# octavian-ganea/equidock_public

Measured on NVIDIA H100. Metric: protein_pairs_per_sec_iegmn_fwd_kabsch, higher is better.
Workload: dtype f32

## Files before the change

equidock_public_b200/csrc/attn_tc.cu:

```cuda
#include "tc_common.cuh"

namespace eqd {

#ifdef ATTN_PROF
__device__ long long g_attn_prof[16];
#define PROF_MARK(k) do { if (tid == 0 && blockIdx.x == 0) { const long long t_ = clock64(); prof_acc[k] += t_ - prof_t; prof_t = t_; } } while (0)
#else
#define PROF_MARK(k) do { } while (0)
#endif

#define AT_THREADS 256
#define AT_KEYS 64
#define AT_CHUNK_BYTES 8192
#define AT_A_SPLIT 16384
#define AT_LD 68

template <bool X5>
struct AtGroupSmem {
  unsigned char k[2][3][AT_CHUNK_BYTES];
  unsigned char v[2][3][AT_CHUNK_BYTES];
  float red[EQD_TM * 2];
  float x5c[X5 ? 2 : 1][X5 ? AT_KEYS * 16 : 4];
  float red5[X5 ? EQD_TM * 2 * 5 : 4];
};
template <bool X5>
struct AtSmem {
  unsigned char qa[3 * AT_A_SPLIT];
  unsigned char pa[3 * AT_A_SPLIT];
  AtGroupSmem<X5> grp;
  unsigned long long k_bar[2], v_bar[2];
};

template <bool X5>
__global__ void __launch_bounds__(AT_THREADS, 1)
attention_tc_kernel(eqd_graph g, const float* __restrict__ proj, int pw, const unsigned char* __restrict__ kv,
                    long kv_split_stride, const float* __restrict__ x5, float* __restrict__ mu, int ldmu) {
  extern __shared__ __align__(128) unsigned char smem_raw[];
  AtSmem<X5>& S = *reinterpret_cast<AtSmem<X5>*>(smem_raw);
  const int tid = threadIdx.x, q = tid, half = q >> 7, r = q & 127, wgi = tid >> 7;
  AtGroupSmem<X5>& G = S.grp;
  TRACE_START(1);
  if (tid == 0) {
    for (int b = 0; b < 2; ++b) {
      mbar_init(&S.k_bar[b], 1);
      mbar_init(&S.v_bar[b], 1);
    }
    asm volatile("fence.mbarrier_init.release.cluster;" ::: "memory");
  }
  if (q == 0) TRACE_PHASE(1, blockIdx.x, 0, 14);
  __syncthreads();
  if (q == 0) TRACE_PHASE(1, blockIdx.x, 0, 13);
  const unsigned k_saddr = smem_u32(G.k), v_saddr = smem_u32(G.v);
  const unsigned qa_saddr = smem_u32(S.qa), pa_saddr = smem_u32(S.pa);
  float* const dtile = reinterpret_cast<float*>(S.pa);
  unsigned kph[2] = {0, 0}, vph[2] = {0, 0};
  const int B = g.n_pairs;
  const unsigned char* k_g = kv;
  const unsigned char* v_g = kv + 3 * kv_split_stride;

  auto load_chunk = [&](const unsigned char* src, unsigned char (*dst)[AT_CHUNK_BYTES], unsigned long long* bar, int blk0,
                        int x5buf) {
    if (q == 0) {
      const bool with5 = X5 && x5buf >= 0;
      mbar_expect_tx(bar, 3 * AT_CHUNK_BYTES + (with5 ? AT_KEYS * 64 : 0));
#pragma unroll
      for (int s = 0; s < 3; ++s) bulk_g2s(dst[s], src + s * kv_split_stride + (long)blk0 * 1024, AT_CHUNK_BYTES, bar);
      if (with5) bulk_g2s(G.x5c[x5buf], x5 + (long)blk0 * 8 * 16, AT_KEYS * 64, bar);
    }
  };
  auto add_s5 = [&](float (&s)[32], const float* xc, const float (&q5)[5]) {
#pragma unroll
    for (int i = 0; i < 32; ++i) {
      const float* row = xc + (half * 32 + i) * 16;
      const float4 k4 = *reinterpret_cast<const float4*>(row);
      const float k8 = row[8];
      s[i] += q5[0] * k4.x + q5[1] * k4.y + q5[2] * k4.z + q5[3] * k4.w + q5[4] * k8;
    }
  };
  auto gemm_s = [&](int kb_, bool hi_only) {
    float d[32];
    wg_gemm6<64>(d, [&](int sp, int kb) { return a_desc_at<EQD_TM>(qa_saddr, AT_A_SPLIT, wgi, sp, kb); },
                 [&](int sp, int kk) { return b_desc_ex(k_saddr + (kb_ * 3 + sp) * AT_CHUNK_BYTES + kk * 256, 128, 1024); },
                 4, false, hi_only);
    wg_store_d<64>(dtile + wgi * 64 * AT_LD, AT_LD, d, tid & 127);
  };
  auto gemm_pv = [&](int vb_) {
    float d[32];
    wg_gemm6<64, 1>(d, [&](int sp, int kb) { return a_desc_at<EQD_TM>(pa_saddr, AT_A_SPLIT, wgi, sp, kb); },
                    [&](int sp, int kk) { return b_desc_ex(v_saddr + (vb_ * 3 + sp) * AT_CHUNK_BYTES + kk * 2048, 1024, 128); },
                    4, false);
    __syncthreads();
    wg_store_d<64>(dtile + wgi * 64 * AT_LD, AT_LD, d, tid & 127);
  };

#ifdef ATTN_PROF
  __shared__ long long prof_acc[16];
  long long prof_t = clock64();
  if (tid == 0)
    for (int k = 0; k < 16; ++k) prof_acc[k] = 0;
#endif
  for (int tile = blockIdx.x; tile < g.n_node_tiles; tile += gridDim.x) {
    PROF_MARK(15);
    if (q == 0) TRACE_PHASE(1, blockIdx.x, tile, 1);
    const int seg = g.node_tiles[2 * tile], node0 = g.node_tiles[2 * tile + 1];
    const int nvalid = min(EQD_TM, g.seg_ptr[seg + 1] - node0);
    const int pseg = seg < B ? seg + B : seg - B;
    const int j0 = g.seg_ptr[pseg], j1 = g.seg_ptr[pseg + 1];
    const int blk_lo = j0 >> 3, blk_hi = (j1 + 7) >> 3;
    const int nchunks = (blk_hi - blk_lo + 7) >> 3;
    const int node = node0 + r;
    const bool valid = r < nvalid;
    PROF_MARK(0);
    if (nchunks > 0) load_chunk(k_g, G.k[0], &S.k_bar[0], blk_lo, 0);
    float q5[5] = {0.f, 0.f, 0.f, 0.f, 0.f};
    if (X5 && valid) {
#pragma unroll
      for (int e = 0; e < 5; ++e) q5[e] = x5[(long)node * 16 + 10 + e];
    }
    {
      float v[32];
      const float4* sp = reinterpret_cast<const float4*>(proj + (long)node * pw + 128 + half * 32);
#pragma unroll
      for (int c4 = 0; c4 < 8; ++c4) {
        float4 t = valid ? sp[c4] : make_float4(0.f, 0.f, 0.f, 0.f);
        v[c4 * 4] = t.x; v[c4 * 4 + 1] = t.y; v[c4 * 4 + 2] = t.z; v[c4 * 4 + 3] = t.w;
      }
      store_half_split3<EQD_TM>(S.qa, AT_A_SPLIT, r, half * 32, v);
    }
    tc_fence_before();
    __syncthreads();
    PROF_MARK(1);
    float mx = -INFINITY;
    for (int c = 0; c < nchunks; ++c) {
      const int kb_ = c & 1;
      if (q == 0) TRACE_PHASE(1, blockIdx.x, tile, (c << 4) | 2);
      mbar_wait(&S.k_bar[kb_], kph[kb_]);
      kph[kb_] ^= 1;
      PROF_MARK(2);
      if (c + 1 < nchunks) load_chunk(k_g, G.k[kb_ ^ 1], &S.k_bar[kb_ ^ 1], blk_lo + 8 * (c + 1), kb_ ^ 1);
      else load_chunk(k_g, G.k[kb_ ^ 1], &S.k_bar[kb_ ^ 1], blk_lo, kb_ ^ 1);
      if (q == 0) TRACE_PHASE(1, blockIdx.x, tile, (c << 4) | 3);
      gemm_s(kb_, true);
      __syncthreads();
      PROF_MARK(3);
      float s[32];
      tile_ld32f(dtile, AT_LD, r, half * 32, s);
      if (X5) add_s5(s, G.x5c[kb_], q5);
      const int key0 = (blk_lo + 8 * c) * 8 + half * 32;
#pragma unroll
      for (int i = 0; i < 32; ++i) {
        int kn = key0 + i;
        mx = fmaxf(mx, (kn >= j0 && kn < j1) ? s[i] : -INFINITY);
      }
      __syncthreads();
      PROF_MARK(4);
    }
    G.red[r * 2 + half] = mx;
    __syncthreads();
    mx = fmaxf(G.red[r * 2], G.red[r * 2 + 1]);
    float l = 0.f;
    float o_acc[32];
#pragma unroll
    for (int i = 0; i < 32; ++i) o_acc[i] = 0.f;
    if (nchunks > 0) load_chunk(v_g, G.v[0], &S.v_bar[0], blk_lo, -1);
    float o5[5] = {0.f, 0.f, 0.f, 0.f, 0.f};
    for (int c = 0; c < nchunks; ++c) {
      const int kb_ = (nchunks + c) & 1, vb_ = c & 1;
      if (q == 0) TRACE_PHASE(1, blockIdx.x, tile, (c << 4) | 4);
      mbar_wait(&S.k_bar[kb_], kph[kb_]);
      kph[kb_] ^= 1;
      PROF_MARK(5);
      if (c + 1 < nchunks) {
        load_chunk(k_g, G.k[kb_ ^ 1], &S.k_bar[kb_ ^ 1], blk_lo + 8 * (c + 1), kb_ ^ 1);
        load_chunk(v_g, G.v[vb_ ^ 1], &S.v_bar[vb_ ^ 1], blk_lo + 8 * (c + 1), -1);
      }
      if (q == 0) TRACE_PHASE(1, blockIdx.x, tile, (c << 4) | 5);
      gemm_s(kb_, false);
      __syncthreads();
      PROF_MARK(6);
      float s[32];
      tile_ld32f(dtile, AT_LD, r, half * 32, s);
      if (X5) add_s5(s, G.x5c[kb_], q5);
      const int key0 = (blk_lo + 8 * c) * 8 + half * 32;
      float l4[4] = {0.f, 0.f, 0.f, 0.f};
#pragma unroll
      for (int i = 0; i < 32; ++i) {
        int kn = key0 + i;
        float pj = (kn >= j0 && kn < j1) ? expf(s[i] - mx) : 0.f;
        s[i] = pj;
        l4[i & 3] += pj;
        if (X5) {
          const float* row = G.x5c[kb_] + (half * 32 + i) * 16;
          const float4 v4 = *reinterpret_cast<const float4*>(row + 4);
          o5[0] = fmaf(pj, v4.x, o5[0]);
          o5[1] = fmaf(pj, v4.y, o5[1]);
          o5[2] = fmaf(pj, v4.z, o5[2]);
          o5[3] = fmaf(pj, v4.w, o5[3]);
          o5[4] = fmaf(pj, row[9], o5[4]);
        }
      }
      l += (l4[0] + l4[1]) + (l4[2] + l4[3]);
      PROF_MARK(7);
      __syncthreads();
      PROF_MARK(8);
      store_half_split3<EQD_TM>(S.pa, AT_A_SPLIT, r, half * 32, s);
      tc_fence_before();
      __syncthreads();
      PROF_MARK(9);
      if (q == 0) TRACE_PHASE(1, blockIdx.x, tile, (c << 4) | 6);
      mbar_wait(&S.v_bar[vb_], vph[vb_]);
      vph[vb_] ^= 1;
      gemm_pv(vb_);
      __syncthreads();
      if (q == 0) TRACE_PHASE(1, blockIdx.x, tile, (c << 4) | 7);
      PROF_MARK(10);
      {
        float oc[32];
        tile_ld32f(dtile, AT_LD, r, half * 32, oc);
#pragma unroll
        for (int i = 0; i < 32; ++i) o_acc[i] += oc[i];
      }
      __syncthreads();
      PROF_MARK(11);
    }
    G.red[r * 2 + half] = l;
    if (X5) {
#pragma unroll
      for (int e = 0; e < 5; ++e) G.red5[(r * 2 + half) * 5 + e] = o5[e];
    }
    __syncthreads();
    l = G.red[r * 2] + G.red[r * 2 + 1];
    {
      const float inv = l > 0.f ? 1.f / l : 0.f;
      if (X5 && valid && half == 0) {
        float e8[8];
#pragma unroll
        for (int e = 0; e < 5; ++e) e8[e] = (G.red5[r * 10 + e] + G.red5[r * 10 + 5 + e]) * inv;
        e8[5] = e8[6] = e8[7] = 0.f;
        float4* de = reinterpret_cast<float4*>(mu + (long)node * ldmu + 64);
        de[0] = make_float4(e8[0], e8[1], e8[2], e8[3]);
        de[1] = make_float4(e8[4], e8[5], e8[6], e8[7]);
      }
      if (valid) {
        float4* dst = reinterpret_cast<float4*>(mu + (long)node * ldmu + half * 32);
#pragma unroll
        for (int c4 = 0; c4 < 8; ++c4)
          dst[c4] = make_float4(o_acc[c4 * 4] * inv, o_acc[c4 * 4 + 1] * inv, o_acc[c4 * 4 + 2] * inv, o_acc[c4 * 4 + 3] * inv);
      }
    }
    __syncthreads();
    PROF_MARK(12);
  }
#ifdef ATTN_PROF
  if (tid == 0 && blockIdx.x == 0)
    for (int k = 0; k < 16; ++k) g_attn_prof[k] = prof_acc[k];
#endif
  if (q == 0) TRACE_PHASE(1, blockIdx.x, 0xffff, 15);
  TRACE_END(1);
}

}

EQD_TRACE_SETTER(eqd_trace_set_attn)

#ifdef ATTN_PROF
extern "C" int eqd_attn_prof_read(long long* out16) {
  return (int)cudaMemcpyFromSymbol(out16, eqd::g_attn_prof, sizeof(long long) * 16);
}
#endif

template <bool X5>
static int launch_attention_tc(const eqd_graph* g, const float* proj, int pw, const void* kv, const float* x5, float* mu,
                               int ldmu, void* stream) {
  if (reinterpret_cast<uintptr_t>(kv) & 15) return EQD_ERR_BAD_ARG;
  if (g->n_node_tiles <= 0) return EQD_OK;
  size_t smem = sizeof(eqd::AtSmem<X5>) + 128;
  EQD_SET_SMEM((eqd::attention_tc_kernel<X5>), smem);
  int grid = g->n_node_tiles < EQD_SMS ? g->n_node_tiles : EQD_SMS;
  long split_stride = (long)((g->n_nodes + 7) / 8 + 8) * 1024;
  eqd::attention_tc_kernel<X5><<<grid, AT_THREADS, smem, (cudaStream_t)stream>>>(
      *g, proj, pw, reinterpret_cast<const unsigned char*>(kv), split_stride, x5, mu, ldmu);
  EQD_CUDA_LAUNCH_CHECK();
  return EQD_OK;
}

extern "C" int eqd_attention_tc(const eqd_graph* g, const float* proj, const void* kv, float* mu, void* stream) {
  if (!g || !proj || !kv || !mu) return EQD_ERR_BAD_ARG;
  return launch_attention_tc<false>(g, proj, 320, kv, nullptr, mu, EQD_HID, stream);
}

extern "C" int eqd_attention_tc0(const eqd_graph* g, const float* proj, const void* kv, const float* x5, float* mu,
                                 void* stream) {
  if (!g || !proj || !kv || !x5 || !mu) return EQD_ERR_BAD_ARG;
  if (reinterpret_cast<uintptr_t>(x5) & 15) return EQD_ERR_BAD_ARG;
  return launch_attention_tc<true>(g, proj, 128 + 3 * 72, kv, x5, mu, EQD_H0_PAD, stream);
}
```

equidock_public_b200/csrc/edge_stage_tc.cu:

```cuda
#include "tc_common.cuh"

namespace eqd {
#define TC_WGS 3
#define TC_THREADS (128 * TC_WGS)
#define TC_ROWS 64
#define TC_MAX_TN 32
#define TC_LD 72
#define TC_W_BYTES 67584
#define TC_W1_SPLIT 6144
#define TC_W23_BASE 18432
#define TC_W23_SPLIT 16384
#define TC_HE_FLOATS (TC_ROWS * EQD_EDGE_FEATS + 16)
#define TC_A_SPLIT 6144

struct __align__(128) TcWgSmem {
  unsigned char a[3 * TC_A_SPLIT];
  float msg[TC_ROWS * TC_LD];
  float he[TC_HE_FLOATS];
  double xs[2][TC_ROWS * 6];
  double xm[TC_ROWS * 3];
  double phi[TC_ROWS];
  int src[2][TC_ROWS];
  int dst[2][TC_ROWS];
  int rp[2][TC_MAX_TN + 4];
  unsigned long long he_bar;
};

struct EdgeConsts {
  float ln_g[64], ln_b[64], b2[64], b3[64], w4[64];
};

struct TcSmem {
  unsigned char w[TC_W_BYTES];
  TcWgSmem wg[TC_WGS];
  EdgeConsts cst;
  unsigned long long w_bar;
};

__device__ __forceinline__ float chain_val(const float (&v)[32], const float (&pv)[32], int h, int ch, int c4, int e) {
  const int i = 4 * (4 * ch + (c4 >> 1)) + 2 * h + e;
  const bool own = ((c4 & 1) == 0) == ((threadIdx.x & 2) == 0);
  return own ? v[i] : pv[i];
}

__global__ void __launch_bounds__(TC_THREADS, 1)
edge_stage_tc_kernel(eqd_graph g, eqd_layer_params p, const __grid_constant__ EdgeConsts cst_p,
                     const float* __restrict__ proj, const double* __restrict__ x_in, const double* __restrict__ x_orig,
                     float* __restrict__ aggr, double* __restrict__ x_out, int* __restrict__ status, int tn) {
  extern __shared__ __align__(128) unsigned char smem_raw[];
  TcSmem& S = *reinterpret_cast<TcSmem*>(smem_raw);
  const int tid = threadIdx.x, wgi = tid >> 7, t = tid & 127, r = t & 63, half = t >> 6;
  const int warp = t >> 5, lane = t & 31;
  TcWgSmem& W = S.wg[wgi];
  const EdgeConsts& cst = S.cst;
  const int bar = 1 + wgi;
  const int pw = 128 + 3 * p.dhp;
  const int ntiles = (g.n_nodes + tn - 1) / tn;
  const float slope = p.leaky_slope;

  TRACE_START(0);
  if (tid == 0) {
    mbar_init(&S.w_bar, 1);
    for (int w = 0; w < TC_WGS; ++w) mbar_init(&S.wg[w].he_bar, 1);
    asm volatile("fence.mbarrier_init.release.cluster;" ::: "memory");
    mbar_expect_tx(&S.w_bar, TC_W_BYTES);
    bulk_g2s(S.w, p.w_edge_tc, TC_W_BYTES, &S.w_bar);
  }
  for (int i = tid; i < 5 * 64; i += TC_THREADS) (&S.cst.ln_g[0])[i] = (&cst_p.ln_g[0])[i];
  __syncthreads();
  mbar_wait(&S.w_bar, 0);
  unsigned he_phase = 0;
  const unsigned w_saddr = smem_u32(S.w), a_saddr = smem_u32(W.a);
  auto a_desc = [&](int sp, int kb) { return a_desc_at<TC_ROWS>(a_saddr, TC_A_SPLIT, 0, sp, kb); };

  auto prefetch = [&](int tile, int buf, int e0, int e1, int& off_l, int& n_l, int& off_r) {
    const int n0 = tile * tn, nn = min(tn, g.n_nodes - n0);
// ... 351 lines not shown
```

equidock_public_b200/csrc/proj_tc.cu:

```cuda
#include "tc_common.cuh"

namespace eqd {

#define PJ_LD 68

template <bool L0>
struct PjCfg {
  static constexpr int R = L0 ? 64 : 128;
  static constexpr int THREADS = 2 * R;
  static constexpr int KB = L0 ? 5 : 4;
  static constexpr int GROUP_BYTES = 64 * KB * 16 * 2 * 3;
  static constexpr int SPLIT_BYTES = 64 * KB * 16 * 2;
  static constexpr int X_SPLIT_BYTES = 16 * KB * 16 * 2;
  static constexpr int W_BYTES = 5 * GROUP_BYTES + (L0 ? 3 * X_SPLIT_BYTES : 0);
  static constexpr int A_SPLIT_BYTES = R * KB * 32;
  static constexpr int NGROUPS = L0 ? 6 : 5;
};

struct PjConsts { float b[336]; };

template <bool L0>
struct PjSmem {
  unsigned char w[PjCfg<L0>::W_BYTES];
  unsigned char a[3 * PjCfg<L0>::A_SPLIT_BYTES];
// ... 98 lines not shown
#pragma unroll
      for (int c = 0; c < 32; ++c) {
        float t = v[c] + cst.b[grp * 64 + half * 32 + c];
        v[c] = act ? lrelu(t, slope) : t;
      }
      if (grp < 3 || kv == nullptr) {
        if (L0) {
          if (valid) {
            float4* o = reinterpret_cast<float4*>(proj + (long)node * pw + grp * 64 + half * 32);
#pragma unroll
            for (int c4 = 0; c4 < 8; ++c4) o[c4] = make_float4(v[c4 * 4], v[c4 * 4 + 1], v[c4 * 4 + 2], v[c4 * 4 + 3]);
          }
        } else {
          float* sc = S.d + r * PJ_LD + half * 32;
#pragma unroll
          for (int c4 = 0; c4 < 8; ++c4)
            *reinterpret_cast<float4*>(sc + c4 * 4) = make_float4(v[c4 * 4], v[c4 * 4 + 1], v[c4 * 4 + 2], v[c4 * 4 + 3]);
          __syncwarp();
          float* o = proj + (long)(node0 + wrow0) * pw + grp * 64 + half * 32 + (lane & 7) * 4;
#pragma unroll
          for (int i = 0; i < 8; ++i) {
            const int row = i * 4 + (lane >> 3);
            float4 t = *reinterpret_cast<const float4*>(S.d + (wrow0 + row) * PJ_LD + half * 32 + (lane & 7) * 4);
            if (node0 + wrow0 + row < n_nodes) *reinterpret_cast<float4*>(o + (long)row * pw) = t;
          }
        }
      }
      if (valid && grp >= 3 && kv != nullptr)
        store_kv_blocks(kv + (long)(grp - 3) * 3 * kv_split_stride, kv_split_stride, node, half, v);
      __syncthreads();
    }
    __syncthreads();
  }
  TRACE_END(2);
}

__global__ void kv_blocks_kernel(int n_nodes, const float* __restrict__ proj, int pw, int koff, int voff,
                                 unsigned char* __restrict__ kv, long kv_split_stride) {
  int idx = blockIdx.x * blockDim.x + threadIdx.x;
  int node = idx >> 2, which = (idx >> 1) & 1, half = idx & 1;
  if (node >= n_nodes) return;
  const float4* src = reinterpret_cast<const float4*>(proj + (long)node * pw + (which ? voff : koff) + half * 32);
  float v[32];
#pragma unroll
  for (int c4 = 0; c4 < 8; ++c4) {
    float4 t = src[c4];
    v[c4 * 4] = t.x; v[c4 * 4 + 1] = t.y; v[c4 * 4 + 2] = t.z; v[c4 * 4 + 3] = t.w;
  }
  store_kv_blocks(kv + (long)which * 3 * kv_split_stride, kv_split_stride, node, half, v);
}

}

EQD_TRACE_SETTER(eqd_trace_set_proj)

extern "C" size_t eqd_kv_blocks_bytes(int32_t n_nodes) {
  return (size_t)6 * ((size_t)(n_nodes + 7) / 8 + 8) * 1024;
}

template <bool L0>
static int launch_project_tc(const eqd_graph* g, const eqd_layer* p_l, const float* h, int ldh, float* proj, int pw,
                             void* kv, float* x5, void* stream) {
  const eqd_layer_params* p = &p_l->dev;
  if (!(p->leaky_slope >= 0.f && p->leaky_slope <= 1.f)) return EQD_ERR_UNSUPPORTED;
  if (!p->w_proj_tc || (reinterpret_cast<uintptr_t>(p->w_proj_tc) & 15)) return EQD_ERR_BAD_ARG;
  if (g->n_nodes <= 0) return EQD_OK;
  eqd::PjConsts cst;
  memset(&cst, 0, sizeof(cst));
  memcpy(&cst, p_l->consts.proj_bias, 320 * sizeof(float));
  int ntiles = (g->n_nodes + eqd::PjCfg<L0>::R - 1) / eqd::PjCfg<L0>::R;
  size_t smem = sizeof(eqd::PjSmem<L0>) + 128;
  EQD_SET_SMEM((eqd::project_tc_kernel<L0>), smem);
  int grid = ntiles < EQD_SMS ? ntiles : EQD_SMS;
  long split_stride = (long)((g->n_nodes + 7) / 8 + 8) * 1024;
  eqd::project_tc_kernel<L0><<<grid, eqd::PjCfg<L0>::THREADS, smem, (cudaStream_t)stream>>>(
      g->n_nodes, *p, cst, h, ldh, proj, pw, reinterpret_cast<unsigned char*>(kv), split_stride, x5);
  EQD_CUDA_LAUNCH_CHECK();
  return EQD_OK;
}

extern "C" int eqd_project_tc(const eqd_graph* g, const eqd_layer* p_l, const float* h, float* proj, void* kv,
                              void* stream) {
  const eqd_layer_params* p = p_l ? &p_l->dev : nullptr;
  if (!g || !p || !h || !proj) return EQD_ERR_BAD_ARG;
  if (p->dh != 64 || p->dhp != 64) return EQD_ERR_UNSUPPORTED;
  return launch_project_tc<false>(g, p_l, h, EQD_HID, proj, 320, kv, nullptr, stream);
}

extern "C" int eqd_project_tc0(const eqd_graph* g, const eqd_layer* p_l, const float* h0, float* proj, void* kv,
                               float* x5, void* stream) {
  const eqd_layer_params* p = p_l ? &p_l->dev : nullptr;
  if (!g || !p || !h0 || !proj || !kv || !x5) return EQD_ERR_BAD_ARG;
  if (p->dh != 69 || p->dhp != 72) return EQD_ERR_UNSUPPORTED;
  return launch_project_tc<true>(g, p_l, h0, EQD_H0_PAD, proj, 128 + 3 * 72, kv, x5, stream);
}

extern "C" int eqd_kv_blocks(const eqd_graph* g, const float* proj, int32_t pw, int32_t koff, int32_t voff, void* kv,
                             void* stream) {
  if (!g || !proj || !kv) return EQD_ERR_BAD_ARG;
  if (g->n_nodes <= 0) return EQD_OK;
  long split_stride = (long)((g->n_nodes + 7) / 8 + 8) * 1024;
  int total = g->n_nodes * 4;
  eqd::kv_blocks_kernel<<<(total + 255) / 256, 256, 0, (cudaStream_t)stream>>>(g->n_nodes, proj, pw, koff, voff,
                                                                                reinterpret_cast<unsigned char*>(kv), split_stride);
  EQD_CUDA_LAUNCH_CHECK();
  return EQD_OK;
}
```

equidock_public_b200/csrc/tc_common.cuh:

```cuda
#pragma once
#include "common.cuh"

namespace eqd {

__device__ __forceinline__ unsigned smem_u32(const void* p) { return (unsigned)__cvta_generic_to_shared(p); }

__device__ __forceinline__ void mbar_init(unsigned long long* bar, int count) {
  asm volatile("mbarrier.init.shared::cta.b64 [%0], %1;" ::"r"(smem_u32(bar)), "r"(count));
}
__device__ __forceinline__ void mbar_wait(unsigned long long* bar, unsigned parity) {
  unsigned addr = smem_u32(bar);
  unsigned done = 0;
  while (!done) {
    asm volatile(
        "{\n\t.reg .pred p;\n\t"
        "mbarrier.try_wait.parity.shared::cta.b64 p, [%1], %2;\n\t"
        "selp.u32 %0, 1, 0, p;\n\t}"
        : "=r"(done) : "r"(addr), "r"(parity) : "memory");
  }
}
__device__ __forceinline__ void mbar_expect_tx(unsigned long long* bar, unsigned bytes) {
  asm volatile("mbarrier.arrive.expect_tx.shared::cta.b64 _, [%0], %1;" ::"r"(smem_u32(bar)), "r"(bytes) : "memory");
}
__device__ __forceinline__ void bulk_g2s(void* dst, const void* src, unsigned bytes, unsigned long long* bar) {
// ... 43 lines not shown
        "wgmma.mma_async.sync.aligned.m64n80k16.f32.bf16.bf16 {%0, %1, %2, %3, %4, %5, %6, %7, %8, %9, %10, %11, %12, %13, %14, %15, %16, %17, %18, %19, %20, %21, %22, %23, %24, %25, %26, %27, %28, %29, %30, %31, %32, %33, %34, %35, %36, %37, %38, %39}, %40, %41, p, 1, 1, 0, %43;\n\t}"
        : "+f"(d[0]), "+f"(d[1]), "+f"(d[2]), "+f"(d[3]), "+f"(d[4]), "+f"(d[5]), "+f"(d[6]), "+f"(d[7]), "+f"(d[8]), "+f"(d[9]), "+f"(d[10]), "+f"(d[11]), "+f"(d[12]), "+f"(d[13]), "+f"(d[14]), "+f"(d[15]), "+f"(d[16]), "+f"(d[17]), "+f"(d[18]), "+f"(d[19]), "+f"(d[20]), "+f"(d[21]), "+f"(d[22]), "+f"(d[23]), "+f"(d[24]), "+f"(d[25]), "+f"(d[26]), "+f"(d[27]), "+f"(d[28]), "+f"(d[29]), "+f"(d[30]), "+f"(d[31]), "+f"(d[32]), "+f"(d[33]), "+f"(d[34]), "+f"(d[35]), "+f"(d[36]), "+f"(d[37]), "+f"(d[38]), "+f"(d[39])
        : "l"(a), "l"(b), "r"(scale_d), "n"(TB));
  }
};

template <int N, int TB>
struct WgmmaRS;
template <int TB>
struct WgmmaRS<64, TB> {
  static __device__ __forceinline__ void mma(float (&d)[32], const unsigned (&a)[4], unsigned long long b, int scale_d) {
    asm volatile(
        "{\n\t.reg .pred p;\n\tsetp.ne.b32 p, %37, 0;\n\t"
        "wgmma.mma_async.sync.aligned.m64n64k16.f32.bf16.bf16 {%0, %1, %2, %3, %4, %5, %6, %7, %8, %9, %10, %11, %12, %13, %14, %15, %16, %17, %18, %19, %20, %21, %22, %23, %24, %25, %26, %27, %28, %29, %30, %31}, {%32, %33, %34, %35}, %36, p, 1, 1, %38;\n\t}"
        : "+f"(d[0]), "+f"(d[1]), "+f"(d[2]), "+f"(d[3]), "+f"(d[4]), "+f"(d[5]), "+f"(d[6]), "+f"(d[7]), "+f"(d[8]), "+f"(d[9]), "+f"(d[10]), "+f"(d[11]), "+f"(d[12]), "+f"(d[13]), "+f"(d[14]), "+f"(d[15]), "+f"(d[16]), "+f"(d[17]), "+f"(d[18]), "+f"(d[19]), "+f"(d[20]), "+f"(d[21]), "+f"(d[22]), "+f"(d[23]), "+f"(d[24]), "+f"(d[25]), "+f"(d[26]), "+f"(d[27]), "+f"(d[28]), "+f"(d[29]), "+f"(d[30]), "+f"(d[31])
        : "r"(a[0]), "r"(a[1]), "r"(a[2]), "r"(a[3]), "l"(b), "r"(scale_d), "n"(TB));
  }
};

template <int N, int TB = 0, class AD, class BD>
__device__ __forceinline__ void wg_gemm6_issue(float (&d)[N / 2], AD a_desc, BD b_desc, int kblocks, bool accumulate,
                                               bool hi_only = false) {
  const int pa[6] = {2, 0, 1, 1, 0, 0}, pb[6] = {0, 2, 1, 0, 1, 0};
  asm volatile("wgmma.fence.sync.aligned;" ::: "memory");
  int scale_d = accumulate ? 1 : 0;
#pragma unroll
  for (int pr = hi_only ? 5 : 0; pr < 6; ++pr)
    for (int kb = 0; kb < kblocks; ++kb) {
      Wgmma<N, TB>::mma(d, a_desc(pa[pr], kb), b_desc(pb[pr], kb), scale_d);
      scale_d = 1;
    }
  asm volatile("wgmma.commit_group.sync.aligned;" ::: "memory");
}
template <int M>
__device__ __forceinline__ void wg_mma_wait(float (&d)[M]) {
  asm volatile("wgmma.wait_group.sync.aligned 0;" ::: "memory");
#pragma unroll
  for (int i = 0; i < M; ++i) asm volatile("" : "+f"(d[i])::"memory");
}
template <int N, int TB = 0, class AD, class BD>
__device__ __forceinline__ void wg_gemm6(float (&d)[N / 2], AD a_desc, BD b_desc, int kblocks, bool accumulate,
                                         bool hi_only = false) {
  wg_gemm6_issue<N, TB>(d, a_desc, b_desc, kblocks, accumulate, hi_only);
  asm volatile("wgmma.wait_group.sync.aligned 0;" ::: "memory");
}
template <int N, int KB, int TB = 0, class BD>
__device__ __forceinline__ void wg_gemm6_rs_issue(float (&d)[N / 2], const unsigned (&a)[3][KB][4], BD b_desc, bool accumulate) {
  constexpr int pa[6] = {2, 0, 1, 1, 0, 0}, pb[6] = {0, 2, 1, 0, 1, 0};
  asm volatile("wgmma.fence.sync.aligned;" ::: "memory");
  int scale_d = accumulate ? 1 : 0;
#pragma unroll
  for (int pr = 0; pr < 6; ++pr)
#pragma unroll
    for (int kb = 0; kb < KB; ++kb) {
      WgmmaRS<N, TB>::mma(d, a[pa[pr]][kb], b_desc(pb[pr], kb), scale_d);
      scale_d = 1;
    }
  asm volatile("wgmma.commit_group.sync.aligned;" ::: "memory");
}

template <int R>
__device__ __forceinline__ unsigned long long a_desc_at(unsigned a_saddr, unsigned split_bytes, int wgi, int s, int kb) {
  return b_desc_ex(a_saddr + s * split_bytes + kb * (32 * R) + wgi * 1024, 16 * R, 128);
}
template <int R>
__device__ __forceinline__ void a_store8(unsigned char* a, unsigned split_bytes, int row, int c, const unsigned* p0,
                                         const unsigned* p1, const unsigned* p2) {
  unsigned char* base = a + (c >> 4) * (32 * R) + ((c >> 3) & 1) * (16 * R) + (row >> 3) * 128 + (row & 7) * 16;
  *reinterpret_cast<uint4*>(base) = make_uint4(p0[0], p0[1], p0[2], p0[3]);
  *reinterpret_cast<uint4*>(base + split_bytes) = make_uint4(p1[0], p1[1], p1[2], p1[3]);
  *reinterpret_cast<uint4*>(base + 2 * split_bytes) = make_uint4(p2[0], p2[1], p2[2], p2[3]);
}

template <int N>
__device__ __forceinline__ void wg_store_d(float* tile, int ld, const float (&d)[N / 2], int t) {
  const int row = (t >> 5) * 16 + ((t & 31) >> 2), col = 2 * (t & 3);
#pragma unroll
  for (int j = 0; j < N / 8; ++j) {
    *reinterpret_cast<float2*>(tile + row * ld + 8 * j + col) = make_float2(d[4 * j], d[4 * j + 1]);
    *reinterpret_cast<float2*>(tile + (row + 8) * ld + 8 * j + col) = make_float2(d[4 * j + 2], d[4 * j + 3]);
  }
}

__device__ __forceinline__ unsigned cvt_bf16x2(float hi, float lo) {
  unsigned d;
  asm("cvt.rn.bf16x2.f32 %0, %1, %2;" : "=r"(d) : "f"(hi), "f"(lo));
  return d;
}
__device__ __forceinline__ void split3_pair(float v0, float v1, unsigned& p0, unsigned& p1, unsigned& p2) {
  p0 = cvt_bf16x2(v1, v0);
  const float r0 = v0 - __uint_as_float(p0 << 16), r1 = v1 - __uint_as_float(p0 & 0xFFFF0000u);
  p1 = cvt_bf16x2(r1, r0);
  p2 = cvt_bf16x2(r1 - __uint_as_float(p1 & 0xFFFF0000u), r0 - __uint_as_float(p1 << 16));
}
template <int R>
__device__ __forceinline__ void store_half_split3(unsigned char* a, unsigned split_bytes, int row, int c0, const float (&v)[32]) {
  unsigned p0[16], p1[16], p2[16];
#pragma unroll
  for (int c = 0; c < 16; ++c) split3_pair(v[2 * c], v[2 * c + 1], p0[c], p1[c], p2[c]);
#pragma unroll
  for (int j = 0; j < 4; ++j) a_store8<R>(a, split_bytes, row, c0 + 8 * j, p0 + 4 * j, p1 + 4 * j, p2 + 4 * j);
}
template <int R>
__device__ __forceinline__ void store_extra8_split3(unsigned char* a, unsigned split_bytes, int row, int c0, const float (&t)[8]) {
  unsigned p0[8], p1[8], p2[8];
#pragma unroll
  for (int c = 0; c < 4; ++c) split3_pair(t[2 * c], t[2 * c + 1], p0[c], p1[c], p2[c]);
#pragma unroll
  for (int c = 4; c < 8; ++c) p0[c] = p1[c] = p2[c] = 0u;
  a_store8<R>(a, split_bytes, row, c0, p0, p1, p2);
  a_store8<R>(a, split_bytes, row, c0 + 8, p0 + 4, p1 + 4, p2 + 4);
}
template <int KB>
__device__ __forceinline__ void acc_to_a_split3(const float (&v)[8 * KB], unsigned (&a)[3][KB][4]) {
#pragma unroll
  for (int kb = 0; kb < KB; ++kb)
#pragma unroll
    for (int i = 0; i < 4; ++i) split3_pair(v[8 * kb + 2 * i], v[8 * kb + 2 * i + 1], a[0][kb][i], a[1][kb][i], a[2][kb][i]);
}
__device__ __forceinline__ void wg_barrier(int id) { asm volatile("bar.sync %0, 128;" ::"r"(id) : "memory"); }
__device__ __forceinline__ bool wg_barrier_and(int id, bool pred) {
  unsigned all;
  asm volatile(
      "{\n\t.reg .pred p, q;\n\tsetp.ne.u32 p, %1, 0;\n\t"
      "bar.red.and.pred q, %2, 128, p;\n\tselp.u32 %0, 1, 0, q;\n\t}"
      : "=r"(all) : "r"((unsigned)pred), "r"(id) : "memory");
  return all != 0;
}
__device__ __forceinline__ void tile_ld32f(const float* tile, int ld, int row, int c0, float (&v)[32]) {
  const float4* s = reinterpret_cast<const float4*>(tile + row * ld + c0);
#pragma unroll
  for (int c4 = 0; c4 < 8; ++c4) {
    float4 t = s[c4];
    v[c4 * 4] = t.x; v[c4 * 4 + 1] = t.y; v[c4 * 4 + 2] = t.z; v[c4 * 4 + 3] = t.w;
  }
}

}
```

Baseline: 38400.

## Add 64-row warpgroup-chain attention and projection kernels with register-A wgmma

Replaces the 128-row, 256-thread attention kernel used by the non-X5 layers with a kernel where each 128-thread warpgroup independently processes 64-row half-tiles. Q and P fragments stay in registers (RS wgmma) instead of being staged through shared memory. Each chain prefetches the next tile's Q and K/V while finishing the current one, and uses per-warpgroup named barriers instead of block-wide syncs. The projection kernel gets a similar 64-row two-chain version that overlaps the five weight-group GEMMs. This adds code complexity and keeps two code paths, since the X5 first layer still uses the old kernel.

```diff
diff --git a/equidock_public_b200/csrc/attn_tc.cu b/equidock_public_b200/csrc/attn_tc.cu
--- a/equidock_public_b200/csrc/attn_tc.cu
+++ b/equidock_public_b200/csrc/attn_tc.cu
@@ -15,30 +15,27 @@
 #define AT_A_SPLIT 16384
 #define AT_LD 68
 
-template <bool X5>
 struct AtGroupSmem {
   unsigned char k[2][3][AT_CHUNK_BYTES];
   unsigned char v[2][3][AT_CHUNK_BYTES];
   float red[EQD_TM * 2];
-  float x5c[X5 ? 2 : 1][X5 ? AT_KEYS * 16 : 4];
-  float red5[X5 ? EQD_TM * 2 * 5 : 4];
+  float x5c[2][AT_KEYS * 16];
+  float red5[EQD_TM * 2 * 5];
 };
-template <bool X5>
 struct AtSmem {
   unsigned char qa[3 * AT_A_SPLIT];
   unsigned char pa[3 * AT_A_SPLIT];
-  AtGroupSmem<X5> grp;
+  AtGroupSmem grp;
   unsigned long long k_bar[2], v_bar[2];
 };
 
-template <bool X5>
 __global__ void __launch_bounds__(AT_THREADS, 1)
-attention_tc_kernel(eqd_graph g, const float* __restrict__ proj, int pw, const unsigned char* __restrict__ kv,
+attention0_tc_kernel(eqd_graph g, const float* __restrict__ proj, int pw, const unsigned char* __restrict__ kv,
                     long kv_split_stride, const float* __restrict__ x5, float* __restrict__ mu, int ldmu) {
   extern __shared__ __align__(128) unsigned char smem_raw[];
-  AtSmem<X5>& S = *reinterpret_cast<AtSmem<X5>*>(smem_raw);
+  AtSmem& S = *reinterpret_cast<AtSmem*>(smem_raw);
   const int tid = threadIdx.x, q = tid, half = q >> 7, r = q & 127, wgi = tid >> 7;
-  AtGroupSmem<X5>& G = S.grp;
+  AtGroupSmem& G = S.grp;
   TRACE_START(1);
   if (tid == 0) {
     for (int b = 0; b < 2; ++b) {
@@ -61,7 +58,7 @@
   auto load_chunk = [&](const unsigned char* src, unsigned char (*dst)[AT_CHUNK_BYTES], unsigned long long* bar, int blk0,
                         int x5buf) {
     if (q == 0) {
-      const bool with5 = X5 && x5buf >= 0;
+      const bool with5 = x5buf >= 0;
       mbar_expect_tx(bar, 3 * AT_CHUNK_BYTES + (with5 ? AT_KEYS * 64 : 0));
 #pragma unroll
       for (int s = 0; s < 3; ++s) bulk_g2s(dst[s], src + s * kv_split_stride + (long)blk0 * 1024, AT_CHUNK_BYTES, bar);
@@ -113,7 +110,7 @@
     PROF_MARK(0);
     if (nchunks > 0) load_chunk(k_g, G.k[0], &S.k_bar[0], blk_lo, 0);
     float q5[5] = {0.f, 0.f, 0.f, 0.f, 0.f};
-    if (X5 && valid) {
+    if (valid) {
 #pragma unroll
       for (int e = 0; e < 5; ++e) q5[e] = x5[(long)node * 16 + 10 + e];
     }
@@ -145,7 +142,7 @@
       PROF_MARK(3);
       float s[32];
       tile_ld32f(dtile, AT_LD, r, half * 32, s);
-      if (X5) add_s5(s, G.x5c[kb_], q5);
+      add_s5(s, G.x5c[kb_], q5);
       const int key0 = (blk_lo + 8 * c) * 8 + half * 32;
 #pragma unroll
       for (int i = 0; i < 32; ++i) {
@@ -180,7 +177,7 @@
       PROF_MARK(6);
       float s[32];
       tile_ld32f(dtile, AT_LD, r, half * 32, s);
-      if (X5) add_s5(s, G.x5c[kb_], q5);
+      add_s5(s, G.x5c[kb_], q5);
       const int key0 = (blk_lo + 8 * c) * 8 + half * 32;
       float l4[4] = {0.f, 0.f, 0.f, 0.f};
 #pragma unroll
@@ -189,7 +186,7 @@
         float pj = (kn >= j0 && kn < j1) ? expf(s[i] - mx) : 0.f;
         s[i] = pj;
         l4[i & 3] += pj;
-        if (X5) {
+        {
           const float* row = G.x5c[kb_] + (half * 32 + i) * 16;
           const float4 v4 = *reinterpret_cast<const float4*>(row + 4);
           o5[0] = fmaf(pj, v4.x, o5[0]);
@@ -224,7 +221,7 @@
       PROF_MARK(11);
     }
     G.red[r * 2 + half] = l;
-    if (X5) {
+    {
 #pragma unroll
       for (int e = 0; e < 5; ++e) G.red5[(r * 2 + half) * 5 + e] = o5[e];
     }
@@ -232,7 +229,7 @@
     l = G.red[r * 2] + G.red[r * 2 + 1];
     {
       const float inv = l > 0.f ? 1.f / l : 0.f;
-      if (X5 && valid && half == 0) {
+      if (valid && half == 0) {
         float e8[8];
 #pragma unroll
         for (int e = 0; e < 5; ++e) e8[e] = (G.red5[r * 10 + e] + G.red5[r * 10 + 5 + e]) * inv;
@@ -259,6 +256,206 @@
   TRACE_END(1);
 }
 
+#define AT_CHAINS 2
+
+struct __align__(128) AtChainSmem {
+  unsigned char k[2][3][AT_CHUNK_BYTES];
+  unsigned char v[2][3][AT_CHUNK_BYTES];
+  float qs[64 * 64];
+  unsigned long long k_bar[2], v_bar[2];
+};
+
+struct AtTile {
+  int node0, nvalid;
+  int j0, j1;
+  int blk_lo, nchunks;
+};
+
+__global__ void __launch_bounds__(AT_CHAINS * 128, 1)
+attention64_tc_kernel(eqd_graph g, const float* __restrict__ proj, const unsigned char* __restrict__ kv,
+                      long kv_split_stride, float* __restrict__ mu) {
+  extern __shared__ __align__(128) unsigned char smem_raw[];
+  AtChainSmem& W = reinterpret_cast<AtChainSmem*>(smem_raw)[threadIdx.x >> 7];
+  const int tid = threadIdx.x, wgi = tid >> 7, t = tid & 127, lane = t & 31;
+  const int bar = 1 + wgi;
+  TRACE_START(1);
+  if (t == 0) {
+    for (int b = 0; b < 2; ++b) {
+      mbar_init(&W.k_bar[b], 1);
+      mbar_init(&W.v_bar[b], 1);
+    }
+    asm volatile("fence.mbarrier_init.release.cluster;" ::: "memory");
+  }
+  wg_barrier(bar);
+  const unsigned k_saddr = smem_u32(W.k), v_saddr = smem_u32(W.v);
+  const int B = g.n_pairs, nht = 2 * g.n_node_tiles, hstride = gridDim.x * AT_CHAINS;
+  const unsigned char* k_g = kv;
+  const unsigned char* v_g = kv + 3 * kv_split_stride;
+
+  const int chain = blockIdx.x * AT_CHAINS + wgi;
+  auto find_tile = [&](int k, AtTile& m) {
+    for (; chain + k * hstride < nht; ++k) {
+      const int ht = (chain + k * hstride) ^ (k & 1);
+      const int seg = __ldg(g.node_tiles + 2 * (ht >> 1));
+      m.node0 = __ldg(g.node_tiles + 2 * (ht >> 1) + 1) + 64 * (ht & 1);
+      m.nvalid = min(64, __ldg(g.seg_ptr + seg + 1) - m.node0);
+      if (m.nvalid <= 0) continue;
+      const int pseg = seg < B ? seg + B : seg - B;
+      m.j0 = __ldg(g.seg_ptr + pseg);
+      m.j1 = __ldg(g.seg_ptr + pseg + 1);
+      m.blk_lo = m.j0 >> 3;
+      m.nchunks = (((m.j1 + 7) >> 3) - m.blk_lo + 7) >> 3;
+      return k;
+    }
+    return -1;
+  };
+  unsigned kfill = 0, kcons = 0, vfill = 0, vcons = 0;
+  auto fill = [&](unsigned char (*dst)[3][AT_CHUNK_BYTES], unsigned long long* bars, unsigned& n, const unsigned char* src,
+                  int blk0) {
+    if (t == 0) {
+      unsigned long long* b = &bars[n & 1];
+      mbar_expect_tx(b, 3 * AT_CHUNK_BYTES);
+#pragma unroll
+      for (int s = 0; s < 3; ++s) bulk_g2s(dst[n & 1][s], src + s * kv_split_stride + (long)blk0 * 1024, AT_CHUNK_BYTES, b);
+    }
+    ++n;
+  };
+  auto consume = [&](unsigned long long* bars, unsigned& n) {
+    mbar_wait(&bars[n & 1], (n >> 1) & 1);
+    return (int)((n++) & 1);
+  };
+  auto stage_q = [&](const AtTile& m) { stage_rows64(W.qs, proj, 320, 128, m.node0, m.nvalid, t); };
+
+  const int fr0 = (t >> 5) * 16 + (lane >> 2), fc = 2 * (lane & 3);
+  AtTile cur, nxt;
+  int kt = find_tile(0, cur);
+  bool k_ahead = false, v_ahead = false;
+  if (kt >= 0) stage_q(cur);
+  while (kt >= 0) {
+    if (t == 0) TRACE_PHASE(1, chain, kt, 1);
+    int ktn = -1;
+    bool looked = false;
+    auto look_ahead = [&]() {
+      if (looked) return;
+      looked = true;
+      ktn = find_tile(kt + 1, nxt);
+      if (ktn >= 0) stage_q(nxt);
+    };
+    if (cur.nchunks > 0 && !k_ahead) fill(W.k, W.k_bar, kfill, k_g, cur.blk_lo);
+    cp_async_wait<0>();
+    wg_barrier(bar);
+    unsigned qf[3][4][4];
+    staged_rows_to_a_split3(W.qs, t, qf);
+    wg_barrier(bar);
+    auto k_desc = [&](int kb_) {
+      return [&, kb_](int sp, int kk) { return b_desc_ex(k_saddr + (kb_ * 3 + sp) * AT_CHUNK_BYTES + kk * 256, 128, 1024); };
+    };
+    float mx[2] = {-INFINITY, -INFINITY};
+    for (int c = 0; c < cur.nchunks; ++c) {
+      const int kb_ = consume(W.k_bar, kcons);
+      fill(W.k, W.k_bar, kfill, k_g, cur.blk_lo + (c + 1 < cur.nchunks ? 8 * (c + 1) : 0));
+      float s[32];
+      wg_gemm6_rs_issue<64, 4, 0, true>(s, qf, k_desc(kb_), false);
+      look_ahead();
+      wg_mma_wait(s);
+      const int key0 = (cur.blk_lo + 8 * c) * 8 + fc;
+#pragma unroll
+      for (int j = 0; j < 8; ++j)
+#pragma unroll
+        for (int e = 0; e < 2; ++e) {
+          const int kn = key0 + 8 * j + e;
+          const bool ok = kn >= cur.j0 && kn < cur.j1;
+#pragma unroll
+          for (int h = 0; h < 2; ++h) mx[h] = fmaxf(mx[h], ok ? s[4 * j + 2 * h + e] : -INFINITY);
+        }
+      wg_barrier(bar);
+    }
+    look_ahead();
+#pragma unroll
+    for (int h = 0; h < 2; ++h) {
+      mx[h] = fmaxf(mx[h], __shfl_xor_sync(0xffffffffu, mx[h], 1));
+      mx[h] = fmaxf(mx[h], __shfl_xor_sync(0xffffffffu, mx[h], 2));
+    }
+    float lh[2][2] = {{0.f, 0.f}, {0.f, 0.f}};
+    float o_acc[32];
+#pragma unroll
+    for (int i = 0; i < 32; ++i) o_acc[i] = 0.f;
+    if (cur.nchunks > 0 && !v_ahead) fill(W.v, W.v_bar, vfill, v_g, cur.blk_lo);
+    for (int c = 0; c < cur.nchunks; ++c) {
+      const int kb_ = consume(W.k_bar, kcons);
+      const bool last = c + 1 == cur.nchunks;
+      if (!last) {
+        fill(W.k, W.k_bar, kfill, k_g, cur.blk_lo + 8 * (c + 1));
+        fill(W.v, W.v_bar, vfill, v_g, cur.blk_lo + 8 * (c + 1));
+      } else if (ktn >= 0 && nxt.nchunks > 0) {
+        fill(W.k, W.k_bar, kfill, k_g, nxt.blk_lo);
+        fill(W.v, W.v_bar, vfill, v_g, nxt.blk_lo);
+      }
+      float s[32];
+      wg_gemm6_rs_issue<64, 4>(s, qf, k_desc(kb_), false);
+      wg_mma_wait(s);
+      const int key0 = (cur.blk_lo + 8 * c) * 8 + fc;
+#pragma unroll
+      for (int j = 0; j < 8; ++j)
+#pragma unroll
+        for (int e = 0; e < 2; ++e) {
+          const int kn = key0 + 8 * j + e;
+          const bool ok = kn >= cur.j0 && kn < cur.j1;
+#pragma unroll
+          for (int h = 0; h < 2; ++h) {
+            float& x = s[4 * j + 2 * h + e];
+            x = ok ? expf(x - mx[h]) : 0.f;
+          }
+        }
+      {
+        float ps[32];
+#pragma unroll
+        for (int i = 0; i < 32; ++i) ps[i] = __shfl_xor_sync(0xffffffffu, s[i], 2);
+#pragma unroll
+        for (int h = 0; h < 2; ++h)
+#pragma unroll
+          for (int ch = 0; ch < 2; ++ch) {
+            float s0 = 0.f, s1 = 0.f;
+#pragma unroll
+            for (int c4 = 0; c4 < 8; ++c4) {
+              s0 = __fadd_rn(s0, chain_val(s, ps, h, ch, c4, 0));
+              s1 = __fadd_rn(s1, chain_val(s, ps, h, ch, c4, 1));
+            }
+            const float sp = __fadd_rn(s0, s1);
+            lh[h][ch] = __fadd_rn(lh[h][ch], __fadd_rn(sp, __shfl_xor_sync(0xffffffffu, sp, 1)));
+          }
+      }
+      unsigned pf[3][4][4];
+      acc_to_a_split3<4>(s, pf);
+      const int vb_ = consume(W.v_bar, vcons);
+      float o[32];
+      wg_gemm6_rs_issue<64, 4, 1>(o, pf, [&](int sp, int kk) {
+        return b_desc_ex(v_saddr + (vb_ * 3 + sp) * AT_CHUNK_BYTES + kk * 2048, 1024, 128); }, false);
+      wg_mma_wait(o);
+#pragma unroll
+      for (int i = 0; i < 32; ++i) o_acc[i] = __fadd_rn(o_acc[i], o[i]);
+      wg_barrier(bar);
+    }
+    k_ahead = v_ahead = ktn >= 0 && nxt.nchunks > 0 && cur.nchunks > 0;
+#pragma unroll
+    for (int h = 0; h < 2; ++h) {
+      const float l = __fadd_rn(lh[h][0], lh[h][1]);
+      const float inv = l > 0.f ? 1.f / l : 0.f;
+      const int row = fr0 + 8 * h;
+      if (row < cur.nvalid) {
+        float* dst = mu + (long)(cur.node0 + row) * EQD_HID + fc;
+#pragma unroll
+        for (int j = 0; j < 8; ++j)
+          *reinterpret_cast<float2*>(dst + 8 * j) = make_float2(o_acc[4 * j + 2 * h] * inv, o_acc[4 * j + 2 * h + 1] * inv);
+      }
+    }
+    kt = ktn;
+    cur = nxt;
+  }
+  cp_async_wait<0>();
+  TRACE_END(1);
+}
+
 }
 
 EQD_TRACE_SETTER(eqd_trace_set_attn)
@@ -269,29 +466,33 @@
 }
 #endif
 
-template <bool X5>
-static int launch_attention_tc(const eqd_graph* g, const float* proj, int pw, const void* kv, const float* x5, float* mu,
-                               int ldmu, void* stream) {
+extern "C" int eqd_attention_tc(const eqd_graph* g, const float* proj, const void* kv, float* mu, void* stream) {
+  if (!g || !proj || !kv || !mu) return EQD_ERR_BAD_ARG;
   if (reinterpret_cast<uintptr_t>(kv) & 15) return EQD_ERR_BAD_ARG;
   if (g->n_node_tiles <= 0) return EQD_OK;
-  size_t smem = sizeof(eqd::AtSmem<X5>) + 128;
-  EQD_SET_SMEM((eqd::attention_tc_kernel<X5>), smem);
-  int grid = g->n_node_tiles < EQD_SMS ? g->n_node_tiles : EQD_SMS;
-  long split_stride = (long)((g->n_nodes + 7) / 8 + 8) * 1024;
-  eqd::attention_tc_kernel<X5><<<grid, AT_THREADS, smem, (cudaStream_t)stream>>>(
-      *g, proj, pw, reinterpret_cast<const unsigned char*>(kv), split_stride, x5, mu, ldmu);
+  const size_t smem = AT_CHAINS * sizeof(eqd::AtChainSmem);
+  EQD_SET_SMEM(eqd::attention64_tc_kernel, smem);
+  const int nht = 2 * g->n_node_tiles;
+  int grid = (nht + AT_CHAINS - 1) / AT_CHAINS;
+  if (grid > EQD_SMS) grid = EQD_SMS;
+  const long split_stride = (long)((g->n_nodes + 7) / 8 + 8) * 1024;
+  eqd::attention64_tc_kernel<<<grid, AT_CHAINS * 128, smem, (cudaStream_t)stream>>>(
+      *g, proj, reinterpret_cast<const unsigned char*>(kv), split_stride, mu);
   EQD_CUDA_LAUNCH_CHECK();
   return EQD_OK;
-}
-
-extern "C" int eqd_attention_tc(const eqd_graph* g, const float* proj, const void* kv, float* mu, void* stream) {
-  if (!g || !proj || !kv || !mu) return EQD_ERR_BAD_ARG;
-  return launch_attention_tc<false>(g, proj, 320, kv, nullptr, mu, EQD_HID, stream);
 }
 
 extern "C" int eqd_attention_tc0(const eqd_graph* g, const float* proj, const void* kv, const float* x5, float* mu,
                                  void* stream) {
   if (!g || !proj || !kv || !x5 || !mu) return EQD_ERR_BAD_ARG;
-  if (reinterpret_cast<uintptr_t>(x5) & 15) return EQD_ERR_BAD_ARG;
-  return launch_attention_tc<true>(g, proj, 128 + 3 * 72, kv, x5, mu, EQD_H0_PAD, stream);
-}
+  if ((reinterpret_cast<uintptr_t>(kv) | reinterpret_cast<uintptr_t>(x5)) & 15) return EQD_ERR_BAD_ARG;
+  if (g->n_node_tiles <= 0) return EQD_OK;
+  const size_t smem = sizeof(eqd::AtSmem) + 128;
+  EQD_SET_SMEM(eqd::attention0_tc_kernel, smem);
+  const int grid = g->n_node_tiles < EQD_SMS ? g->n_node_tiles : EQD_SMS;
+  const long split_stride = (long)((g->n_nodes + 7) / 8 + 8) * 1024;
+  eqd::attention0_tc_kernel<<<grid, AT_THREADS, smem, (cudaStream_t)stream>>>(
+      *g, proj, 128 + 3 * 72, reinterpret_cast<const unsigned char*>(kv), split_stride, x5, mu, EQD_H0_PAD);
+  EQD_CUDA_LAUNCH_CHECK();
+  return EQD_OK;
+}
diff --git a/equidock_public_b200/csrc/edge_stage_tc.cu b/equidock_public_b200/csrc/edge_stage_tc.cu
--- a/equidock_public_b200/csrc/edge_stage_tc.cu
+++ b/equidock_public_b200/csrc/edge_stage_tc.cu
@@ -36,12 +36,6 @@
   EdgeConsts cst;
   unsigned long long w_bar;
 };
-
-__device__ __forceinline__ float chain_val(const float (&v)[32], const float (&pv)[32], int h, int ch, int c4, int e) {
-  const int i = 4 * (4 * ch + (c4 >> 1)) + 2 * h + e;
-  const bool own = ((c4 & 1) == 0) == ((threadIdx.x & 2) == 0);
-  return own ? v[i] : pv[i];
-}
 
 __global__ void __launch_bounds__(TC_THREADS, 1)
 edge_stage_tc_kernel(eqd_graph g, eqd_layer_params p, const __grid_constant__ EdgeConsts cst_p,
diff --git a/equidock_public_b200/csrc/proj_tc.cu b/equidock_public_b200/csrc/proj_tc.cu
--- a/equidock_public_b200/csrc/proj_tc.cu
+++ b/equidock_public_b200/csrc/proj_tc.cu
@@ -154,6 +154,126 @@
     }
     __syncthreads();
   }
+  TRACE_END(2);
+}
+
+#define PJ_CHAINS 2
+#define PJ64_W_BYTES (5 * PjCfg<false>::GROUP_BYTES)
+#define PJ_OUT_LD 72
+
+struct __align__(128) PjChainSmem {
+  float hs[64 * 64];
+  float out[64 * PJ_OUT_LD];
+};
+struct Pj64Smem {
+  unsigned char w[PJ64_W_BYTES];
+  PjChainSmem ch[PJ_CHAINS];
+  float b[320];
+  unsigned long long w_bar;
+};
+
+__global__ void __launch_bounds__(PJ_CHAINS * 128, 1)
+project64_tc_kernel(int n_nodes, eqd_layer_params p, const __grid_constant__ PjConsts cst, const float* __restrict__ h,
+                    float* __restrict__ proj, unsigned char* __restrict__ kv, long kv_split_stride) {
+  extern __shared__ __align__(128) unsigned char smem_raw[];
+  Pj64Smem& S = *reinterpret_cast<Pj64Smem*>(smem_raw);
+  const int tid = threadIdx.x, wgi = tid >> 7, t = tid & 127, lane = t & 31;
+  PjChainSmem& W = S.ch[wgi];
+  const int bar = 1 + wgi;
+  const int ntiles = (n_nodes + 63) / 64, tstride = gridDim.x * PJ_CHAINS;
+  TRACE_START(2);
+  if (tid == 0) {
+    mbar_init(&S.w_bar, 1);
+    asm volatile("fence.mbarrier_init.release.cluster;" ::: "memory");
+    mbar_expect_tx(&S.w_bar, PJ64_W_BYTES);
+    bulk_g2s(S.w, p.w_proj_tc, PJ64_W_BYTES, &S.w_bar);
+  }
+  for (int i = tid; i < 320; i += PJ_CHAINS * 128) S.b[i] = cst.b[i];
+  __syncthreads();
+  const unsigned w_saddr = smem_u32(S.w);
+  const float slope = p.leaky_slope;
+  const int fr0 = (t >> 5) * 16 + (lane >> 2), fc = 2 * (lane & 3);
+  auto stage_h = [&](int tile) { stage_rows64(W.hs, h, EQD_HID, 0, (long)tile * 64, min(64, n_nodes - tile * 64), t); };
+  int tile = blockIdx.x * PJ_CHAINS + wgi;
+  if (tile < ntiles) stage_h(tile);
+  mbar_wait(&S.w_bar, 0);
+
+  for (; tile < ntiles; tile += tstride) {
+    if (t == 0) TRACE_PHASE(2, blockIdx.x * PJ_CHAINS + wgi, tile, 1);
+    const int node0 = tile * 64, nvalid = min(64, n_nodes - node0);
+    cp_async_wait<0>();
+    wg_barrier(bar);
+    unsigned af[3][4][4];
+    staged_rows_to_a_split3(W.hs, t, af);
+    wg_barrier(bar);
+    if (tile + tstride < ntiles) stage_h(tile + tstride);
+    auto group = [&](int grp) {
+      return [&, grp](int s, int kb) { return b_desc_ex(w_saddr + grp * PjCfg<false>::GROUP_BYTES + s * PjCfg<false>::SPLIT_BYTES + kb * 2048, 1024, 128); };
+    };
+    float acc[2][32];
+    wg_gemm6_rs_issue<64, 4>(acc[0], af, group(0), false);
+#pragma unroll
+    for (int grp = 0; grp < 5; ++grp) {
+      float (&d)[32] = acc[grp & 1];
+      if (grp + 1 < 5) {
+        wg_gemm6_rs_issue<64, 4>(acc[(grp + 1) & 1], af, group(grp + 1), false);
+        wg_mma_wait<1>(d);
+      } else {
+        wg_mma_wait(d);
+      }
+      const bool act = (grp == 2 || grp == 3);
+#pragma unroll
+      for (int j = 0; j < 8; ++j) {
+        const float2 bj = *reinterpret_cast<const float2*>(&S.b[grp * 64 + 8 * j + fc]);
+#pragma unroll
+        for (int hh = 0; hh < 2; ++hh) {
+          float& x0 = d[4 * j + 2 * hh];
+          float& x1 = d[4 * j + 2 * hh + 1];
+          x0 = x0 + bj.x;
+          x1 = x1 + bj.y;
+          if (act) {
+            x0 = lrelu(x0, slope);
+            x1 = lrelu(x1, slope);
+          }
+        }
+      }
+      if (grp < 3 || kv == nullptr) {
+#pragma unroll
+        for (int j = 0; j < 8; ++j)
+#pragma unroll
+          for (int hh = 0; hh < 2; ++hh)
+            *reinterpret_cast<float2*>(W.out + (fr0 + 8 * hh) * PJ_OUT_LD + 8 * j + fc) =
+                make_float2(d[4 * j + 2 * hh], d[4 * j + 2 * hh + 1]);
+        wg_barrier(bar);
+#pragma unroll
+        for (int i = 0; i < 8; ++i) {
+          const int row = i * 8 + (t >> 4), c4 = t & 15;
+          if (row < nvalid)
+            *reinterpret_cast<float4*>(proj + (long)(node0 + row) * 320 + grp * 64 + 4 * c4) =
+                *reinterpret_cast<const float4*>(W.out + row * PJ_OUT_LD + 4 * c4);
+        }
+        wg_barrier(bar);
+      } else {
+        unsigned char* base = kv + (long)(grp - 3) * 3 * kv_split_stride;
+#pragma unroll
+        for (int hh = 0; hh < 2; ++hh) {
+          const int row = fr0 + 8 * hh, node = node0 + row;
+          if (row < nvalid) {
+            unsigned char* nb = base + (long)(node >> 3) * 1024 + (node & 7) * 16 + fc * 2;
+#pragma unroll
+            for (int j = 0; j < 8; ++j) {
+              unsigned w0, w1, w2;
+              split3_pair(d[4 * j + 2 * hh], d[4 * j + 2 * hh + 1], w0, w1, w2);
+              *reinterpret_cast<unsigned*>(nb + j * 128) = w0;
+              *reinterpret_cast<unsigned*>(nb + kv_split_stride + j * 128) = w1;
+              *reinterpret_cast<unsigned*>(nb + 2 * kv_split_stride + j * 128) = w2;
+            }
+          }
+        }
+      }
+    }
+  }
+  cp_async_wait<0>();
   TRACE_END(2);
 }
 
@@ -206,7 +326,22 @@
   const eqd_layer_params* p = p_l ? &p_l->dev : nullptr;
   if (!g || !p || !h || !proj) return EQD_ERR_BAD_ARG;
   if (p->dh != 64 || p->dhp != 64) return EQD_ERR_UNSUPPORTED;
-  return launch_project_tc<false>(g, p_l, h, EQD_HID, proj, 320, kv, nullptr, stream);
+  if (!(p->leaky_slope >= 0.f && p->leaky_slope <= 1.f)) return EQD_ERR_UNSUPPORTED;
+  if (!p->w_proj_tc || (reinterpret_cast<uintptr_t>(p->w_proj_tc) & 15)) return EQD_ERR_BAD_ARG;
+  if (g->n_nodes <= 0) return EQD_OK;
+  eqd::PjConsts cst;
+  memset(&cst, 0, sizeof(cst));
+  memcpy(&cst, p_l->consts.proj_bias, 320 * sizeof(float));
+  const int ntiles = (g->n_nodes + 63) / 64;
+  const size_t smem = sizeof(eqd::Pj64Smem) + 128;
+  EQD_SET_SMEM(eqd::project64_tc_kernel, smem);
+  int grid = (ntiles + PJ_CHAINS - 1) / PJ_CHAINS;
+  if (grid > EQD_SMS) grid = EQD_SMS;
+  const long split_stride = (long)((g->n_nodes + 7) / 8 + 8) * 1024;
+  eqd::project64_tc_kernel<<<grid, PJ_CHAINS * 128, smem, (cudaStream_t)stream>>>(
+      g->n_nodes, *p, cst, h, proj, reinterpret_cast<unsigned char*>(kv), split_stride);
+  EQD_CUDA_LAUNCH_CHECK();
+  return EQD_OK;
 }
 
 extern "C" int eqd_project_tc0(const eqd_graph* g, const eqd_layer* p_l, const float* h0, float* proj, void* kv,
diff --git a/equidock_public_b200/csrc/tc_common.cuh b/equidock_public_b200/csrc/tc_common.cuh
--- a/equidock_public_b200/csrc/tc_common.cuh
+++ b/equidock_public_b200/csrc/tc_common.cuh
@@ -99,9 +99,9 @@
     }
   asm volatile("wgmma.commit_group.sync.aligned;" ::: "memory");
 }
-template <int M>
+template <int PENDING = 0, int M>
 __device__ __forceinline__ void wg_mma_wait(float (&d)[M]) {
-  asm volatile("wgmma.wait_group.sync.aligned 0;" ::: "memory");
+  asm volatile("wgmma.wait_group.sync.aligned %0;" ::"n"(PENDING) : "memory");
 #pragma unroll
   for (int i = 0; i < M; ++i) asm volatile("" : "+f"(d[i])::"memory");
 }
@@ -111,13 +111,13 @@
   wg_gemm6_issue<N, TB>(d, a_desc, b_desc, kblocks, accumulate, hi_only);
   asm volatile("wgmma.wait_group.sync.aligned 0;" ::: "memory");
 }
-template <int N, int KB, int TB = 0, class BD>
+template <int N, int KB, int TB = 0, bool HI_ONLY = false, class BD>
 __device__ __forceinline__ void wg_gemm6_rs_issue(float (&d)[N / 2], const unsigned (&a)[3][KB][4], BD b_desc, bool accumulate) {
   constexpr int pa[6] = {2, 0, 1, 1, 0, 0}, pb[6] = {0, 2, 1, 0, 1, 0};
   asm volatile("wgmma.fence.sync.aligned;" ::: "memory");
   int scale_d = accumulate ? 1 : 0;
 #pragma unroll
-  for (int pr = 0; pr < 6; ++pr)
+  for (int pr = HI_ONLY ? 5 : 0; pr < 6; ++pr)
 #pragma unroll
     for (int kb = 0; kb < KB; ++kb) {
       WgmmaRS<N, TB>::mma(d, a[pa[pr]][kb], b_desc(pb[pr], kb), scale_d);
@@ -184,6 +184,32 @@
   for (int kb = 0; kb < KB; ++kb)
 #pragma unroll
     for (int i = 0; i < 4; ++i) split3_pair(v[8 * kb + 2 * i], v[8 * kb + 2 * i + 1], a[0][kb][i], a[1][kb][i], a[2][kb][i]);
+}
+__device__ __forceinline__ int stage_swz(int row) { return (row & 3) << 1; }
+__device__ __forceinline__ void stage_rows64(float* rows, const float* src, int ld, int col0, long row0, int nvalid, int t) {
+#pragma unroll
+  for (int i = 0; i < 8; ++i) {
+    const int idx = i * 128 + t, row = idx >> 4, k4 = idx & 15;
+    const bool ok = row < nvalid;
+    cp_async16(rows + row * 64 + ((k4 ^ stage_swz(row)) << 2), src + (row0 + (ok ? row : 0)) * ld + col0 + 4 * k4, ok);
+  }
+  cp_async_commit();
+}
+__device__ __forceinline__ void staged_rows_to_a_split3(const float* rows, int t, unsigned (&a)[3][4][4]) {
+  const int g = (t >> 5) * 16 + ((t & 31) >> 2), c = t & 3;
+#pragma unroll
+  for (int kb = 0; kb < 4; ++kb)
+#pragma unroll
+    for (int i = 0; i < 4; ++i) {
+      const int row = g + 8 * (i & 1), k4 = 4 * kb + 2 * (i >> 1) + (c >> 1);
+      const float2 v = *reinterpret_cast<const float2*>(rows + row * 64 + ((k4 ^ stage_swz(row)) << 2) + 2 * (c & 1));
+      split3_pair(v.x, v.y, a[0][kb][i], a[1][kb][i], a[2][kb][i]);
+    }
+}
+__device__ __forceinline__ float chain_val(const float (&v)[32], const float (&pv)[32], int h, int ch, int c4, int e) {
+  const int i = 4 * (4 * ch + (c4 >> 1)) + 2 * h + e;
+  const bool own = ((c4 & 1) == 0) == ((threadIdx.x & 2) == 0);
+  return own ? v[i] : pv[i];
 }
 __device__ __forceinline__ void wg_barrier(int id) { asm volatile("bar.sync %0, 128;" ::"r"(id) : "memory"); }
 __device__ __forceinline__ bool wg_barrier_and(int id, bool pred) {
```

Result: faster. 41630, median of 6 (+8.4%).
